# graphdeco-inria/reduced-3dgs

Measured on AMD Instinct MI355X. Metric: train iters/s (fwd+bwd) + Mpix/s render, 500k Gaussians @1600x1062, higher is better.
Workload: dtype f32

## Files before the change

reduced-3dgs_amd/csrc/binning.hip:

```cpp
#include <cstdlib>
#include <cstring>
#include <mutex>
#include <string>

#include <rocprim/rocprim.hpp>

#include "depth_sort.h"

namespace r3 {

struct GatherTiles {
    const uint32_t* tiles;
    __host__ __device__ uint32_t operator()(uint32_t id) const { return tiles[id]; }
};

size_t depth_sort_temp_bytes(size_t P)
{
    size_t a = 0, b = 0;
    uint32_t* n = nullptr;
    R3_HIP(rocprim::radix_sort_pairs(nullptr, a, n, n, rocprim::counting_iterator<uint32_t>(0), n, P, 0, 32));
    auto it = rocprim::make_transform_iterator(n, GatherTiles{n});
    R3_HIP(rocprim::inclusive_scan(nullptr, b, it, n, P, rocprim::plus<uint32_t>()));
    return (a > b ? a : b) + 256;
}

void run_generic_depth_sort(int P, GeomState& g, hipStream_t s)
{
    size_t bytes = g.temp_bytes;
    R3_HIP(rocprim::radix_sort_pairs(g.temp, bytes, g.depth_key, g.key_sorted, rocprim::counting_iterator<uint32_t>(0),
                                     g.order, (size_t)P, 0, 32, s));
    bytes = g.temp_bytes;
    auto it = rocprim::make_transform_iterator(g.order, GatherTiles{g.tiles});
    R3_HIP(rocprim::inclusive_scan(g.temp, bytes, it, g.offsets, (size_t)P, rocprim::plus<uint32_t>(), s));
}

__global__ __launch_bounds__(1024) void header_reduce_kernel(const HeaderArgs* __restrict__ ap)
{
    __shared__ uint32_t s_red[16][6];
    const HeaderArgs a = *ap;
    const PrePartial all = reduce_partials(a.parts, a.n_parts, s_red);
    if (threadIdx.x == 0) write_header(a, all);
}
// ... 124 lines not shown
    const uint32_t n = min(j_hi - j_lo + 1u, (uint32_t)kEmitSlice);
    const uint32_t start0 = s_start0;
    auto stage = [&](uint32_t r0, uint32_t nr) {
        for (uint32_t k = threadIdx.x; k < nr; k += 256) {
            const uint32_t g = j_lo + r0 + k, id = a.order[g];
            s_start[k] = r0 + k == 0 ? start0 : offsets[g - 1];
            s_id[k] = id;
            s_rect[k] = a.rect_sorted ? a.rect_sorted[g] : a.rect[id];
        }
    };
    const uint32_t nr0 = min(n, (uint32_t)kEmitStage);
    stage(0u, nr0);
    __syncthreads();
    for (uint32_t k = threadIdx.x; k < n; k += 256) {
        const uint32_t start = k < nr0 ? s_start[k] : offsets[j_lo + k - 1];
        a.rec[k < nr0 ? s_id[k] : a.order[j_lo + k]].pair_start = start;
        if (start >= pos0) s_owner[start - pos0] = (unsigned short)k;
    }
    __syncthreads();
    {
        constexpr int E = kEmitPerBlock / 256;
        const int lane = threadIdx.x & 63, w = threadIdx.x >> 6;
        uint32_t v[E];
#pragma unroll
        for (int i = 0; i < E; i++) v[i] = s_owner[threadIdx.x * E + i];
#pragma unroll
        for (int i = 1; i < E; i++) v[i] = max(v[i], v[i - 1]);
        uint32_t incl = v[E - 1];
        for (int off = 1; off < 64; off <<= 1) {
            const uint32_t up = (uint32_t)__shfl_up((int)incl, off);
            if (lane >= off) incl = max(incl, up);
// ... 354 lines not shown
```

reduced-3dgs_amd/csrc/blend.hip:

```cpp
#include <cstdlib>

#include "blend_math.h"
#include "common.h"

namespace r3 {

constexpr int kChunk = 64;

#if defined(R3_TIMELINE) || defined(R3_TIMELINE_FWD)
__device__ unsigned long long g_timeline[4 * 65536];
#define R3_TL_BEGIN_(id) const unsigned long long tl0_ = __builtin_amdgcn_s_memtime(); const uint32_t tlid_ = (id);
#define R3_TL_END_(extra)                                                                                                \
    if (threadIdx.x == 0 && tlid_ < 65536u) {                                                                            \
        g_timeline[4 * tlid_] = tl0_;                                                                                     \
        g_timeline[4 * tlid_ + 1] = __builtin_amdgcn_s_memtime();                                                         \
        g_timeline[4 * tlid_ + 2] = (unsigned long long)__builtin_amdgcn_s_getreg((4 << 0) | (0 << 6) | (31 << 11)) |     \
                                    ((unsigned long long)__builtin_amdgcn_s_getreg((20 << 0) | (0 << 6) | (31 << 11)) << 32); \
        g_timeline[4 * tlid_ + 3] = (unsigned long long)(extra);                                                          \
    }
#endif
#if defined(R3_TIMELINE)
#define R3_TL_BEGIN(id) R3_TL_BEGIN_(id)
#define R3_TL_END(extra) R3_TL_END_(extra)
#else
// ... 533 lines not shown
                {
                    typedef float v4f __attribute__((ext_vector_type(4)));
                    const volatile v4f __attribute__((address_space(3)))* zp =
                        (const volatile v4f __attribute__((address_space(3)))*)reinterpret_cast<float*>(s_zero);
                    const v4f z0 = zp[0], z1 = zp[1];
                    const float z2 = *(const volatile float __attribute__((address_space(3)))*)(zp + 2);
                    sg.sx = z0.x; sg.sy = z0.y; sg.sxx = z0.z; sg.sxy = z0.w;
                    sg.syy = z1.x; sg.sm = z1.y; sg.r = z1.z; sg.g = z1.w; sg.b = z2;
                }
#else
                sg.sx = sg.sy = sg.sxx = sg.sxy = sg.syy = sg.sm = sg.r = sg.g = sg.b = 0.f;
#endif
            }
        }
        __syncthreads();
        if (lane < n && ((contributed >> lane) & 1ull)) {
            const float4 c = s_rec[lane].c;
            const uint32_t rect_min = __float_as_uint(c.y), width = __float_as_uint(c.z) & 0xffffu;
            const uint32_t slot = __float_as_uint(c.w) + ((uint32_t)tile_y - (rect_min >> 16)) * width +
                                  ((uint32_t)tile_x - (rect_min & 0xffffu));
            float4* dst = reinterpret_cast<float4*>(a.pair_grad + (size_t)slot * kPairStride);
            const float* src = s_grad + lane * kGradStride;
            SplatSums u;
            u.sx = src[0];
            u.sy = src[1];
            u.sxx = src[2];
            u.sxy = src[3];
            u.syy = src[4];
            u.sm = src[5];
            u.r = src[6];
            u.g = src[7];
            u.b = src[8];
            const SplatGrad g = splat_grad_of(load_splat(s_rec[lane]), u);
            dst[0] = make_float4(g.mx * half_w, g.my * half_h, g.cA, g.cB);
            dst[1] = make_float4(g.cC, g.op, g.r, g.g);
            dst[2] = make_float4(g.b, 0.f, 0.f, 0.f);
            if (kPairStride >= 16) dst[3] = make_float4(0.f, 0.f, 0.f, 0.f);
            a.pair_flag[slot] = 1;
        }
    }
    R3_TL_END(hi - lo)
}

#if defined(R3_TIMELINE) || defined(R3_TIMELINE_FWD)
extern "C" int r3dgs_debug_timeline(unsigned long long* host, int n)
{
    return (int)hipMemcpyFromSymbol(host, HIP_SYMBOL(g_timeline), sizeof(unsigned long long) * 4 * (size_t)n);
}
#endif

constexpr int kOrderThreads = 1024, kOrderClasses = 1024;

__device__ __forceinline__ uint32_t unit_segments(uint32_t list_len, uint32_t deepest, uint32_t thr, uint32_t walk)
// ... 254 lines not shown
```

reduced-3dgs_amd/csrc/capi.hip:

```cpp
#include "../../include/r3dgs_rasterizer.h"
#include "../../include/r3dgs_quantised.h"

#include <time.h>

#include <atomic>
#include <random>
#include <chrono>
#include <cmath>
#include <cstddef>
#include <cstdlib>
#include <cstring>
#include <deque>
#include <map>
#include <mutex>
#include <unordered_map>
#include <vector>

#include "common.h"
#include "quant_math.h"

namespace r3 {
int env_int(const char* env, int dflt, int lo, int hi)
{
    const char* v = getenv(env);
// ... 397 lines not shown
    }
}

template <class Block>
void launch_write_args(Block* dst, const Block& v, hipStream_t s);

template <class Hooks>
void issue_backward(const BwdPlan& p, BwdPassArgs* d, const BwdPassArgs& args, hipStream_t s, Hooks& h)
{
    h.begin(kBlendBwd, s);
    if (p.has_pairs) {
        issue_unit_order(p, d, args, s);
        h.begin(kBlendBwdKernel, s);
        issue_blend_backward(p, d, args, s);
        h.end(kBlendBwdKernel, "blend backward kernel", s);
        issue_pair_reduce(p, &d->reduce, s);
    } else {
        launch_write_args(d, args, s);
    }
    h.end(kBlendBwd, "blend backward", s);
    h.begin(kPreBwd, s);
    issue_preprocess_backward(p, &d->pre, s);
    h.end(kPreBwd, "preprocess backward", s);
}

template <class Block>
void launch_write_args(Block* dst, const Block& v, hipStream_t s)
{
    hipLaunchKernelGGL(write_args_kernel<Block>, dim3(1), dim3(256), 0, s, dst, v);
}

// ... 193 lines not shown
    d.hist_rows = g.hist_rows;
    d.hist_base = g.hist_base;
    d.key_sorted = g.key_sorted;
    d.bucket_id = g.bucket_id;
    d.ovf_key = g.ovf_key;
    d.ovf_id = g.ovf_id;
    d.rect = g.rect;
    d.rec16 = g.rec16;
    d.rec16_b = g.rec16_b;
    d.rect_sorted = g.rect_sorted;
    d.order = g.order;
    d.offsets = g.offsets;
    uint32_t* const block_first = (b && fuse_header && !p.generic_depth_sort) ? b->block_first : nullptr;
    d.block_first = block_first;
    d.block_cap = p.reserve / (uint32_t)kRadixBlock + 2u;

    const PairLayout& l = p.layout;
    const size_t Tn = (size_t)p.gx * p.gy;
    if (b) {
        const uint32_t stride = radix_row_stride(p.reserve);
        EmitArgs& e = a.emit;
        e.P = c.P;
        e.gx = p.gx;
        e.hdr = g.header;
        e.order = g.order;
        e.offsets = g.offsets;
        e.block_first = block_first;
        e.rect = g.rect;
        e.rect_sorted = p.generic_depth_sort ? nullptr : g.rect_sorted;
        e.rec = g.rec;
// ... 539 lines not shown
        bb.W = width;
        bb.H = height;
        bb.gx = plan.gx;
        bb.nblocks = (uint32_t)(plan.gx * plan.gy * (4 / plan.bwd_ppl));
        bb.bg = background;
        bb.pair_grad = bin.pair_grad;
        bb.pair_flag = bin.pair_flag;
        bb.quad_masks = binning_buffer && keep_quad_masks() ? bin.quad_masks : nullptr;
        bb.tile_order = (heaviest_tiles_first() && plan.has_pairs && (size_t)plan.gx * plan.gy <= ((size_t)1 << kUnitTileBits))
                            ? bin.unit_order : nullptr;
        bb.units_cap = plan.units_cap;
        bb.quad_depth = img.quad_depth;
        bb.ckpt = plan.has_pairs ? bin.ckpt : nullptr;
        bb.hdr = geom.header;
        bb.segments = bwd_segments();
        PairReduceArgs& pr = a.reduce;
        pr.hdr = geom.header;
        pr.pair_grad = bin.pair_grad;
        pr.pair_flag = bin.pair_flag;
        pr.pair_rank = bin.pair_rank;
        pr.rank_mask = plan.layout.wide ? 0xFFFFFFFFu : (1u << plan.layout.rank_bits) - 1u;
        pr.order = nullptr;
        pr.rec = geom.rec;
        pr.tiles = geom.tiles;
        pr.acc = geom.acc;
        pr.wave_part = bin.wave_part;
        {
            static std::atomic<unsigned long long> stamp{[] {
                std::random_device rd;
                return ((unsigned long long)rd() << 32) ^ (unsigned long long)rd() ^ 0x9E3779B97F4A7C15ull;
            }()};
            const unsigned long long st = stamp.fetch_add(1);
            pr.stamp0 = (uint32_t)st;
            pr.stamp1 = (uint32_t)(st >> 32);
        }
        PreBwdArgs& pb = a.pre;
        FwdInputs& in = pb.in;
        in.P = P;
        in.M = M;
        in.degrees = D;
        in.means3D = means3D;
        in.scales = scales;
        in.rotations = rotations;
        in.opacities = nullptr;
        in.shs = colors_precomp ? nullptr : shs;
        in.cov3D_precomp = cov3D_precomp;
        in.colors_precomp = colors_precomp;
        ViewParams& view = pb.view;
        view.view = viewmatrix;
        view.proj = projmatrix;
        view.campos = campos;
        view.bg = background;
        view.tan_fovx = tan_fovx;
        view.tan_fovy = tan_fovy;
        view.W = width;
        view.H = height;
        view.scale_modifier = scale_modifier;
        pb.radii = radii;
        pb.rec = geom.rec;
        pb.tiles = geom.tiles;
        pb.acc = geom.acc;
        pb.wave_part = plan.has_pairs ? bin.wave_part : nullptr;
        pb.stamp0 = pr.stamp0;
        pb.stamp1 = pr.stamp1;
        pb.header = geom.header;
        pb.lambda_sh = lambda_sh_sparsity;
        pb.sh_ddir = (lambda_sh_sparsity == 0.f && sh_derivative_cache()) ? geom.sh_ddir : nullptr;
        pb.out.dL_dmean2D = dL_dmean2D;
        pb.out.dL_dopacity = dL_dopacity;
        pb.out.dL_dcolor = dL_dcolor;
        pb.out.dL_dmean3D = dL_dmean3D;
        pb.out.dL_dcov3D = dL_dcov3D;
        pb.out.dL_dsh = dL_dsh;
        pb.shs_rest = raw ? shs_rest : nullptr;
        pb.dL_dsh_rest = raw ? dL_dsh_rest : nullptr;
        pb.out.dL_dscale = dL_dscale;
        pb.out.dL_drot = dL_drot;
        pb.out.dL_dconic = dL_dconic;
        {
// ... 331 lines not shown
```

reduced-3dgs_amd/csrc/common.h:

```cpp
#pragma once
#include <hip/hip_runtime.h>
#include <stddef.h>
#include <stdint.h>

#include <functional>
#include <stdexcept>
#include <string>

#include "gauss_math.h"
#include "param_math.h"

namespace r3 {

constexpr size_t kAlign = 256;
constexpr int kPairGrad = 9;
constexpr int kPieceStride = 9;
constexpr int kAccStride = 12;
constexpr int kPairStride = 12;
static_assert(kAccStride >= 12 && kAccStride % 4 == 0 && kPairStride >= 12 && kPairStride % 4 == 0,
              "the kernels move three float4 per row");

constexpr int kPreBlockSize = 256;
struct PrePartial {
    uint32_t visible;
    uint32_t num_rendered;
    uint32_t depth_max;
    uint32_t depth_inv_min;
    uint32_t binned;
    uint32_t rendered_ref;
    uint32_t pad[2];
};
static_assert(sizeof(PrePartial) == 32, "two 16-byte loads per partial");
struct GeomHeader {
    uint32_t visible, num_rendered, depth_max, depth_inv_min;
    uint32_t num_pairs;
// ... 60 lines not shown
    {
        T* r = reinterpret_cast<T*>(p);
        size_t bytes = (count * sizeof(T) + kAlign - 1) & ~(kAlign - 1);
        p += bytes;
        return r;
    }
};

struct GeomState {
    GeomHeader* header;
    PrePartial* partials;
    DepthSortScratch* dsort;
    unsigned long long* hist_rows;
    uint32_t* hist_base;
    GRec* rec;
    float* acc;
    ushort4* rect;
    uint32_t* depth_key;
    uint32_t* tiles;
    uint32_t* key_sorted;
    uint32_t* bucket_id;
    uint4* rec16;
    ushort4* rect_sorted;
    uint4* rec16_b;
    uint32_t* order;
    uint32_t* offsets;
    int* radii_internal;
    float* sh_ddir;
    uint32_t* ovf_key;
    uint32_t* ovf_id;
    char* temp;
    size_t temp_bytes;
    static GeomState carve(char* base, size_t P, size_t temp_bytes)
    {
        Carver c(base);
        GeomState g;
        const size_t nb = (size_t)depth_bucket_count(P);
        g.header = c.take<GeomHeader>(1);
        g.partials = c.take<PrePartial>(pre_partials(P));
        g.dsort = c.take<DepthSortScratch>(1);
        g.hist_rows = c.take<unsigned long long>(depth_hist_rows(P) * (nb + 1));
        g.hist_base = c.take<uint32_t>(depth_hist_rows(P) * (nb + 1));
        g.rec = c.take<GRec>(P);
        g.acc = c.take<float>(P * kAccStride);
        g.rect = c.take<ushort4>(P);
        g.depth_key = c.take<uint32_t>(P);
        g.tiles = c.take<uint32_t>(P);
        g.key_sorted = c.take<uint32_t>(P);
        g.bucket_id = c.take<uint32_t>(P);
        g.order = c.take<uint32_t>(P);
        g.offsets = c.take<uint32_t>(P);
        g.radii_internal = c.take<int>(P);
        g.ovf_key = c.take<uint32_t>(P);
        g.ovf_id = c.take<uint32_t>(P);
        g.rec16 = c.take<uint4>(P);
        g.rect_sorted = c.take<ushort4>(P);
        g.rec16_b = c.take<uint4>(P);
        g.temp = c.take<char>(temp_bytes);
        g.temp_bytes = temp_bytes;
// ... 66 lines not shown
        return (uint32_t)(m < n() ? m : n());
    }
};
R3_HD uint32_t bwd_list_fit(uint32_t pairs, const TileGrid& g)
{
    const size_t extra = (size_t)pairs >> kBwdSegMinLog2, most = 8 * g.n();
    return g.list_tiles_max() + (uint32_t)((extra < most ? extra : most) / kOrderLists);
}
inline uint32_t bwd_units_cap(uint32_t reserve, const TileGrid& g) { return (bwd_list_fit(reserve, g) + 1u) * kOrderLists; }
int bwd_segment_log2();
int bwd_segment_factor_pct();

struct BinState {
    uint32_t* point_list;
    float* pair_grad;
    float* wave_part;
    unsigned char* pair_flag;
    uint32_t* pair_rank;
    char* words_a;
    char* words_b;
    char* words_c;
    uint32_t* radix_rows;
    uint32_t* radix_base;
    uint32_t* radix_total;
    uint32_t* block_first;
    unsigned long long* quad_masks;
    uint32_t* unit_order;
    float4* ckpt;
    char* end;
    static BinState carve(char* base, size_t R, int wide, const TileGrid& grid)
    {
        const size_t Tn = grid.n();
        Carver c(base);
        BinState b;
        b.point_list = c.take<uint32_t>(R);
        b.pair_grad = c.take<float>(R * kPairStride);
        b.wave_part = c.take<float>((R / 64 + 1) * 2 * kPieceStride);
        b.pair_flag = c.take<unsigned char>(R);
        if (wide == 1) {
            b.pair_rank = c.take<uint32_t>(R);
            b.words_a = reinterpret_cast<char*>(c.take<unsigned long long>(R));
            b.words_b = reinterpret_cast<char*>(c.take<unsigned long long>(R));
            b.words_c = nullptr;
        } else if (wide == 2) {
            b.words_a = reinterpret_cast<char*>(c.take<unsigned long long>(R));
            b.words_b = reinterpret_cast<char*>(c.take<unsigned long long>(R));
            b.words_c = nullptr;
            b.pair_rank = reinterpret_cast<uint32_t*>(b.words_a);
        } else {
            b.words_a = reinterpret_cast<char*>(c.take<uint32_t>(R));
            b.words_b = reinterpret_cast<char*>(c.take<uint32_t>(R));
            b.words_c = reinterpret_cast<char*>(c.take<uint32_t>(R));
// ... 193 lines not shown
    DepthSortScratch* ds;
    unsigned long long* hist_rows;
    uint32_t* hist_base;
    uint32_t* key_sorted;
    uint32_t* bucket_id;
    uint32_t* ovf_key;
    uint32_t* ovf_id;
    const ushort4* rect;
    uint4* rec16;
    uint4* rec16_b;
    ushort4* rect_sorted;
    uint32_t* order;
    uint32_t* offsets;
    uint32_t* block_first;
    uint32_t block_cap;
};
struct EmitArgs {
    int P, gx;
    const GeomHeader* hdr;
    const uint32_t* order;
    const uint32_t* offsets;
    const uint32_t* block_first;
    const ushort4* rect;
    const ushort4* rect_sorted;
    GRec* rec;
    int rank_bits, digit_bits;
    char* words_out;
    uint32_t cap;
    uint32_t* pair_rank;
    uint2* ranges;
// ... 49 lines not shown
    const uint32_t* n_contrib;
    const float* dL_dpix;
    int W, H, gx;
    uint32_t nblocks;
    const float* bg;
    float* pair_grad;
    unsigned char* pair_flag;
    const unsigned long long* quad_masks;
    uint32_t* tile_order;
    uint32_t units_cap;
    const uint32_t* quad_depth;
    const float4* ckpt;
    const GeomHeader* hdr;
    int segments;
};
struct PairReduceArgs {
    const GeomHeader* hdr;
    const float* pair_grad;
    unsigned char* pair_flag;
    const uint32_t* pair_rank;
    uint32_t rank_mask;
    const uint32_t* order;
    const GRec* rec;
    const uint32_t* tiles;
    float* acc;
    float* wave_part;
    uint32_t stamp0, stamp1;
};
struct PreBwdArgs {
    FwdInputs in;
    ViewParams view;
    const int* radii;
    const GRec* rec;
    const uint32_t* tiles;
    const float* acc;
    const float* wave_part;
    uint32_t stamp0, stamp1;
    const GeomHeader* header;
    float lambda_sh;
    const float* sh_ddir;
    int stagger;
    BwdOutputs out;
    const float* shs_rest;
    float* dL_dsh_rest;
};

struct FwdPassArgs {
    PreArgs pre;
    HeaderArgs header;
    DepthArgs depth;
    EmitArgs emit;
    RadixArgs radix[kMaxRadixPasses];
    RangesArgs ranges;
    BlendFwdArgs blend;
    const float* shs_rest;
    QuantInputs quant;
};
struct BwdPassArgs {
    BlendBwdArgs blend;
    PairReduceArgs reduce;
    PreBwdArgs pre;
};
static_assert(sizeof(FwdPassArgs) <= 3072 && sizeof(BwdPassArgs) <= 3072, "pass blocks travel as by-value kernel arguments");

struct FwdPlan {
    int P, M, W, H, gx, gy;
    uint32_t reserve;
    uint32_t grid_pairs;
    PairLayout layout;
    int nb;
    int ragged, counters;
    int color_grid;
    int color_split[3];
    int generic_depth_sort;
    int tight;
// ... 24 lines not shown
                             int* degrees, hipStream_t s);

void issue_header_reduce(const HeaderArgs* a, hipStream_t s);
void prepare_depth_bucket_sort(int nb);
void issue_depth_sort_and_color(const FwdPlan& p, const FwdPassArgs* a, hipStream_t s);
void run_generic_depth_sort(int P, GeomState& g, hipStream_t s);
void issue_tile_binning(const FwdPlan& p, const FwdPassArgs* a, hipStream_t s);
const char* sorted_words(const BinState& b, const PairLayout& l);
void launch_export_keys(int P, int R, int cap, size_t n_tiles, const BinState& b, const GeomState& g, uint64_t* keys_out,
                        hipStream_t s);
void launch_export_point_list(int count, const uint32_t* point_list, const GeomHeader* hdr, uint32_t* out, hipStream_t s);

void issue_blend_forward(const FwdPlan& p, const BlendFwdArgs* a, hipStream_t s);
void issue_unit_order(const BwdPlan& p, BwdPassArgs* dst, const BwdPassArgs& v, hipStream_t s);
void issue_blend_backward(const BwdPlan& p, BwdPassArgs* dst, const BwdPassArgs& v, hipStream_t s);
void issue_pair_reduce(const BwdPlan& p, const PairReduceArgs* a, hipStream_t s);
void issue_preprocess_backward(const BwdPlan& p, const PreBwdArgs* a, hipStream_t s);

void launch_colour_variance_accumulate(int P, const int* D, int M, int max_sh_deg, const float* means3D,
                                       const float* cam_pos, const float* shs, const int* radii, const int* touched,
                                       const float* transmittance, float* wSum, float* wSumSq, float* mean,
                                       float* variance, float* accum, hipStream_t s);

int env_int(const char* env, int dflt, int lo, int hi);

#if defined(__HIPCC__)
template <class Block>
__device__ __forceinline__ void install_block_from_kernarg(Block* dst, int tid, int nthreads)
{
    static_assert(alignof(Block) == 8 && sizeof(Block) % 4 == 0, "kernarg layout: [dst (8 B)][block]");
#if defined(__HIP_DEVICE_COMPILE__)
// ... 10 lines not shown
```

reduced-3dgs_amd/csrc/depth_sort.h:

```cpp
#pragma once
#include "common.h"

namespace r3 {

template <class T>
__device__ inline T block256_inclusive_scan(T v, T* s_w)
{
    const int lane = threadIdx.x & 63, w = threadIdx.x >> 6;
    for (int off = 1; off < 64; off <<= 1) {
        const T up = __shfl_up(v, off);
        if (lane >= off) v += up;
    }
    __syncthreads();
    if (lane == 63) s_w[w] = v;
    __syncthreads();
    T add = 0;
    for (int k = 0; k < w; k++) add += s_w[k];
    return v + add;
}

template <int BITS>
__device__ __forceinline__ unsigned long long match_digit(uint32_t d, bool valid)
{
    unsigned long long peers = __ballot(valid);
#pragma unroll
    for (int b = 0; b < BITS; b++) {
        const bool bit = (d >> b) & 1u;
        const unsigned long long bal = __ballot(bit);
        peers &= bit ? bal : ~bal;
    }
    return peers;
}

constexpr int kWaveSortMax = 512;
constexpr int kGlobalSplitMax = 64;
constexpr uint32_t kGlobalSplitCap = kGlobalSplitMax * 2048u;
constexpr int kBucketsPerGroup = 4;
constexpr int kHistPerThread = kHistBatch / 256;
constexpr int kCountBits = 24;
constexpr unsigned long long kCountMask = (1ull << kCountBits) - 1;

__device__ __forceinline__ void publish_offset(const DepthArgs& a, uint32_t slot, uint32_t end, uint32_t count)
{
    a.offsets[slot] = end;
    if (a.block_first && count) {
        const uint32_t first = end - count;
        for (uint32_t m = (first + (uint32_t)kRadixBlock - 1u) / (uint32_t)kRadixBlock;
// ... 203 lines not shown
    unsigned long long run = block256_inclusive_scan(sum, s_tmp) - sum;
    for (int k = 0; k < per; k++) {
        const int b = b0 + k;
        if (b <= nb + 1) {
            s_start[b] = (uint32_t)(run & kCountMask);
            if (publish) {
                ds->start[b] = (uint32_t)(run & kCountMask);
                ds->tile_base[b] = (uint32_t)(run >> kCountBits);
            }
            run += b <= nb ? ds->total[b] : 0ull;
        }
    }
    __syncthreads();
}

__device__ inline void depth_scatter_role(const DepthArgs& a, char* smem, int wg)
{
    const int P = a.P, nb = a.nb;
    unsigned long long* s_tmp = reinterpret_cast<unsigned long long*>(smem);
    uint32_t* slot0 = reinterpret_cast<uint32_t*>(smem + 256 * sizeof(unsigned long long));
    uint32_t* rank = slot0 + (nb + 2);
    scan_bucket_totals(a.ds, nb, slot0, s_tmp, wg == 0);
    if (wg == 0 && threadIdx.x == 0 && a.info) {
        volatile PassInfo* info = a.info;
        info->sort_overflow = a.hdr->sort_overflow;
        __threadfence_system();
        info->sort_seq = a.ticket;
    }
    const uint32_t R = a.hdr->num_rendered;
    const uint32_t* mybase = a.hist_base + (size_t)wg * (nb + 1);
    for (int b = threadIdx.x; b <= nb; b += 256) {
        slot0[b] += mybase[b];
        rank[b] = 0;
    }
    const DepthRange rng = make_depth_range(a.hdr->depth_max, a.hdr->depth_inv_min, nb);
    __syncthreads();
    const uint2* __restrict__ rects = reinterpret_cast<const uint2*>(a.rect);
    for (int base = wg * a.per_block; base < min(P, (wg + 1) * a.per_block); base += kHistBatch) {
        uint32_t kv[kHistPerThread];
        uint2 rv[kHistPerThread];
#pragma unroll
        for (int k = 0; k < kHistPerThread; k++) {
            const int i = base + k * 256 + threadIdx.x;
            kv[k] = i < P ? a.key[i] : 0xFFFFFFFFu;
            rv[k] = i < P ? rects[i] : make_uint2(0u, 0u);
        }
#pragma unroll
        for (int k = 0; k < kHistPerThread; k++) {
            const uint32_t id = (uint32_t)(base + k * 256 + threadIdx.x);
            if ((int)id < P) {
                const int b = depth_bucket(kv[k], rng);
                const uint32_t slot = slot0[b] + atomicAdd(&rank[b], 1u);
                if (b == nb) {
                    a.order[slot] = id;
                    a.offsets[slot] = R;
                } else {
                    a.rec16[slot] = make_uint4(kv[k], id, rv[k].x, rv[k].y);
                }
            }
        }
// ... 482 lines not shown
```

reduced-3dgs_amd/csrc/preprocess_bwd.hip:

```cpp
#include "common.h"

namespace r3 {

constexpr int kBwdBlock = 64;
constexpr int kBwdWaveShFloats = 64 * 48 + (64 * 48) / 32;

template <bool ROWS48>
__device__ __forceinline__ int bskew(int e)
{
    if (ROWS48) return e + (int)(((uint32_t)e * 43691u) >> 21);
    return e + (e >> 5);
}

template <bool ROWS48>
struct ShRowLdsRW {
    float* base;
    int roff;
    __device__ __forceinline__ float at(int e) const { return ROWS48 ? base[e] : base[bskew<false>(roff + e)]; }
    __device__ __forceinline__ void put(int e, float v) const
    {
        if (ROWS48)
            base[e] = v;
        else
            base[bskew<false>(roff + e)] = v;
// ... 55 lines not shown
            for (int e4 = lane; e4 < n4; e4 += 64) {
                const int f = e4 << 2;
                dst4[e4] = make_float4(lds[split_lds_index<ROWS48>(f, rl, k0, M)], lds[split_lds_index<ROWS48>(f + 1, rl, k0, M)],
                                       lds[split_lds_index<ROWS48>(f + 2, rl, k0, M)], lds[split_lds_index<ROWS48>(f + 3, rl, k0, M)]);
            }
        } else {
            for (int e4 = lane; e4 < n4; e4 += 64) dst4[e4] = make_float4(0.f, 0.f, 0.f, 0.f);
        }
    } else if (rows) {
        for (int f = lane; f < len; f += 64) dst[f] = lds[split_lds_index<ROWS48>(f, rl, k0, M)];
    } else {
        for (int f = lane; f < len; f += 64) dst[f] = 0.f;
    }
}

constexpr int kReduceGroups = 1;

__device__ __forceinline__ void pair_reduce_group(const PairReduceArgs& a, uint32_t e, int lane, bool valid, uint32_t key,
                                                  float (&v)[kPairGrad], uint32_t key_before, uint32_t key_after)
{
#define R3_SEG_STEP(CTRL, RMASK)                                                                                          \
    {                                                                                                                     \
        const uint32_t ku = (uint32_t)__builtin_amdgcn_update_dpp((int)~key, (int)key, CTRL, RMASK, 0xf, false);          \
        const bool take = ku == key;                                                                                      \
        _Pragma("unroll") for (int k = 0; k < kPairGrad; k++)                                                             \
        {                                                                                                                 \
            const float vu = __builtin_bit_cast(                                                                          \
                float, __builtin_amdgcn_update_dpp(0, __builtin_bit_cast(int, v[k]), CTRL, RMASK, 0xf, false));           \
            if (take) v[k] += vu;                                                                                         \
        }                                                                                                                 \
    }
    R3_SEG_STEP(0x111, 0xf)
    R3_SEG_STEP(0x112, 0xf)
    R3_SEG_STEP(0x114, 0xf)
    R3_SEG_STEP(0x118, 0xf)
    R3_SEG_STEP(0x142, 0xa)
    R3_SEG_STEP(0x143, 0xc)
#undef R3_SEG_STEP
    const uint32_t knext = (uint32_t)__shfl_down((int)key, 1);
    const uint32_t key0 = (uint32_t)__builtin_amdgcn_readfirstlane((int)key);
    if (valid && (lane == 63 || knext != key)) {
        const uint32_t gid = a.order ? global_ptr(a.order)[key] : key;
        const bool from_before = key == key0 && key_before == key;
        const bool into_next = lane == 63 && key_after == key;
        if (!from_before && !into_next) {
            auto* dst = reinterpret_cast<R3_GLOBAL float4*>(global_ptr(a.acc) + (size_t)gid * kAccStride);
            bool nz = false;
#pragma unroll
            for (int k = 0; k < kPairGrad; k++) nz |= v[k] != 0.f;
            if (nz) {
                dst[0] = make_float4(v[0], v[1], v[2], v[3]);
                dst[1] = make_float4(v[4], v[5], v[6], v[7]);
                dst[2] = make_float4(v[8], __uint_as_float(a.stamp0), __uint_as_float(a.stamp1), 0.f);
            }
        } else {
            R3_GLOBAL float* wp = global_ptr(a.wave_part) + (size_t)(e >> 6) * 2 * kPieceStride;
            if (from_before) {
#pragma unroll
                for (int k = 0; k < kPairGrad; k++) wp[k] = v[k];
            }
            if (into_next) {
#pragma unroll
                for (int k = 0; k < kPairGrad; k++) wp[kPieceStride + k] = v[k];
            }
        }
    }
}

__global__ __launch_bounds__(256) void pair_reduce_kernel(const PairReduceArgs* __restrict__ ap)
{
    const PairReduceArgs a = *ap;
    const uint32_t R = global_ptr(a.hdr)->num_pairs;
    constexpr uint32_t kPerBlock = 256u * kReduceGroups;
  for (uint32_t blk = blockIdx.x; blk * kPerBlock < R; blk += gridDim.x) {
    const R3_GLOBAL float* __restrict__ pair_grad = global_ptr(a.pair_grad);
    R3_GLOBAL unsigned char* __restrict__ pair_flag = global_ptr(a.pair_flag);
    const R3_GLOBAL uint32_t* __restrict__ pair_gid = global_ptr(a.pair_rank);
    const uint32_t rank_mask = a.rank_mask;
    const int lane = threadIdx.x & 63, wave = threadIdx.x >> 6;
    const uint32_t e0 = blk * kPerBlock + (uint32_t)wave * (64u * kReduceGroups) + (uint32_t)lane;
    float v[kReduceGroups][kPairGrad];
    uint32_t key[kReduceGroups], kb[kReduceGroups], ka[kReduceGroups];
    bool flag[kReduceGroups];
#pragma unroll
    for (int g = 0; g < kReduceGroups; g++) {
        const uint32_t e = e0 + 64u * g, gbase = e & ~63u;
        key[g] = e < R ? pair_gid[e] & rank_mask : 0xFFFFFFFFu;
        flag[g] = e < R && pair_flag[e] != 0;
        kb[g] = gbase > 0u && gbase < R ? pair_gid[gbase - 1u] & rank_mask : 0xFFFFFFFFu;
        ka[g] = gbase + 64u < R ? pair_gid[gbase + 64u] & rank_mask : 0xFFFFFFFFu;
    }
#pragma unroll
    for (int g = 0; g < kReduceGroups; g++) {
        const uint32_t e = e0 + 64u * g;
#pragma unroll
        for (int k = 0; k < kPairGrad; k++) v[g][k] = 0.f;
        if (flag[g]) {
            pair_flag[e] = 0;
            const auto* src = reinterpret_cast<const R3_GLOBAL float4*>(pair_grad + (size_t)e * kPairStride);
            const float4 r0 = src[0], r1 = src[1];
            v[g][0] = r0.x; v[g][1] = r0.y; v[g][2] = r0.z; v[g][3] = r0.w;
            v[g][4] = r1.x; v[g][5] = r1.y; v[g][6] = r1.z; v[g][7] = r1.w;
            v[g][8] = src[2].x;
        }
    }
#pragma unroll
    for (int g = 0; g < kReduceGroups; g++) {
        const uint32_t e = e0 + 64u * g;
        pair_reduce_group(a, e, lane, e < R, key[g], v[g], kb[g], ka[g]);
    }
  }
}

void issue_pair_reduce(const BwdPlan& p, const PairReduceArgs* a, hipStream_t s)
{
    if (!p.has_pairs) return;
    constexpr uint32_t per = 256u * kReduceGroups;
    hipLaunchKernelGGL(pair_reduce_kernel, dim3((p.grid_pairs + per - 1u) / per), dim3(256), 0, s, a);
}

template <bool ROWS48, bool F64, bool RAW = false>
__global__ __launch_bounds__(kBwdBlock) void preprocess_bwd_kernel(const PreBwdArgs* __restrict__ ap)
{
    __shared__ float s_sh[kBwdBlock / 64][kBwdWaveShFloats];
    const PreBwdArgs a = *ap;
    const int tid = threadIdx.x, lane = tid & 63, wave = tid >> 6;
    const int P = a.in.P, M = a.in.M;
    const int i = blockIdx.x * kBwdBlock + tid;
    const bool valid = i < P;
    const int wave_first = blockIdx.x * kBwdBlock + wave * 64;
    const Camera cam = load_camera_from(global_ptr(a.view.view), global_ptr(a.view.proj), global_ptr(a.view.campos), a.view);
    const bool has_sh = a.in.shs != nullptr;
    const auto* hdr = global_ptr(a.header);
    const uint32_t num_pairs = hdr->num_pairs, n_visible = hdr->visible, hdr_sh_cache = hdr->sh_cache;
    const bool cached = has_sh && a.sh_ddir != nullptr && hdr_sh_cache != 0u;

    int radius = 0, deg = 0;
    uint32_t ntile = 0u;
    GRec r;
    float4 a0, a1, a2;
    float m3[3], sc[3], q[4], c6[6], d9in[9];
    const auto load_lane = [&]() {
        r = global_ptr(a.rec)[i];
        ntile = global_ptr(a.tiles)[i];
        const auto* arow = reinterpret_cast<const R3_GLOBAL float4*>(global_ptr(a.acc) + (size_t)i * kAccStride);
        a0 = arow[0];
        a1 = arow[1];
        a2 = arow[2];
        for (int k = 0; k < 3; k++) m3[k] = global_ptr(a.in.means3D)[3 * i + k];
        if (!a.in.cov3D_precomp) {
            for (int k = 0; k < 3; k++) sc[k] = global_ptr(a.in.scales)[3 * i + k];
            for (int k = 0; k < 4; k++) q[k] = global_ptr(a.in.rotations)[4 * i + k];
        }
        if (has_sh) deg = global_ptr(a.in.degrees)[i];
        if (cached) {
#pragma unroll
            for (int k = 0; k < 9; k++) d9in[k] = global_ptr(a.sh_ddir)[9 * (size_t)i + k];
        }
        if (a.in.cov3D_precomp) {
            for (int k = 0; k < 6; k++) c6[k] = global_ptr(a.in.cov3D_precomp)[6 * i + k];
            sc[0] = sc[1] = sc[2] = 0.f;
            q[0] = 1.f;
            q[1] = q[2] = q[3] = 0.f;
        }
    };
    if (valid) radius = global_ptr(a.radii)[i];
    const bool vis = valid && radius > 0;
    if (vis) load_lane();

    const int nrows = max(0, min(64, P - wave_first));
    const int span_len = has_sh ? nrows * 3 * M : 0;
    const long span_first = 3L * M * wave_first;
    float* lds = s_sh[wave];
    const bool wave_vis = __ballot(vis) != 0ull;
    if (!cached && a.stagger > 0 && blockIdx.x < 768u * (256 / kBwdBlock)) {
        const int steps = (int)(blockIdx.x / (256u * (256 / kBwdBlock))) * a.stagger;
        for (int k = 0; k < steps; k += 127) __builtin_amdgcn_s_sleep(127);
    }
    if (RAW) {
        if (wave_vis && !cached) {
            const int rl = 3 * (M - 1);
            const auto* dc = global_ptr(a.in.shs) + 3L * wave_first;
            const auto* rest = global_ptr(a.shs_rest) + (long)rl * wave_first;
// ... 40 lines not shown
                }
            }
        } else {
            for (int e = lane; e < span_len; e += 64) lds[bskew<ROWS48>(e)] = src[e];
        }
    }
    __syncthreads();

    float dmean[3] = {0.f, 0.f, 0.f}, dcov6[6] = {0.f, 0.f, 0.f, 0.f, 0.f, 0.f};
    float dscale[3] = {0.f, 0.f, 0.f}, dq[4] = {0.f, 0.f, 0.f, 0.f};
    float g2x = 0.f, g2y = 0.f, dop = 0.f, dcol[3] = {0.f, 0.f, 0.f}, gcon[3] = {0.f, 0.f, 0.f};
    int K = 0;
    const ShRowLdsRW<ROWS48> row{ROWS48 ? lds + 49 * lane : lds, ROWS48 ? 0 : lane * 3 * M};
    if (vis) {
        const float mx = m3[0], my = m3[1], mz = m3[2];
        const uint32_t start = r.pair_start;
        if (a.wave_part && start != 0xFFFFFFFFu && start + ntile <= num_pairs) {
            float acc9[kPairGrad];
            const uint32_t last = start + ntile - 1u;
            const uint32_t w0 = start >> 6, w1 = last >> 6;
            if (w0 == w1) {
                if (__float_as_uint(a2.y) != a.stamp0 || __float_as_uint(a2.z) != a.stamp1)
                    a0 = a1 = a2 = make_float4(0.f, 0.f, 0.f, 0.f);
                acc9[0] = a0.x; acc9[1] = a0.y; acc9[2] = a0.z; acc9[3] = a0.w;
                acc9[4] = a1.x; acc9[5] = a1.y; acc9[6] = a1.z; acc9[7] = a1.w;
                acc9[8] = a2.x;
            } else {
                const R3_GLOBAL float* wave_part = global_ptr(a.wave_part);
                const R3_GLOBAL float* wp = wave_part + (size_t)w0 * 2 * kPieceStride + kPieceStride;
#pragma unroll
                for (int k = 0; k < kPairGrad; k++) acc9[k] = wp[k];
                for (uint32_t w = w0 + 1; w <= w1; w++) {
                    wp = wave_part + (size_t)w * 2 * kPieceStride;
#pragma unroll
                    for (int k = 0; k < kPairGrad; k++) acc9[k] += wp[k];
                }
            }
            g2x = acc9[0];
            g2y = acc9[1];
            gcon[0] = acc9[2];
            gcon[1] = acc9[3];
            gcon[2] = acc9[4];
            dop = acc9[5];
            dcol[0] = acc9[6];
            dcol[1] = acc9[7];
            dcol[2] = acc9[8];
        }
        float qn = 1.f;
        if (!a.in.cov3D_precomp) {
            if (RAW) {
                const float rq[4] = {q[0], q[1], q[2], q[3]};
                for (int k = 0; k < 3; k++) sc[k] = scale_act(sc[k]);
                qn = quat_act(rq, q);
            }
            cov3d_from_scale_rot(sc, cam.scale_modifier, q, c6);
        }
        double dcov6d[6];
        if (F64) {
            cov2d_backward_f64(cam, mx, my, mz, c6, gcon[0], gcon[1], gcon[2], dcov6d, dmean);
#pragma unroll
            for (int k = 0; k < 6; k++) dcov6[k] = (float)dcov6d[k];
        } else {
// ... 141 lines not shown
```

Baseline: 1588.

## Fold per-pair gradient reduction into preprocess backward via slab-ordered pair layout

Removes the separate pair_reduce kernel and its per-Gaussian acc buffer, wave_part spill and stamp scheme. Pair slots are now assigned in Gaussian-index order: a prefix scan over tile counts runs inside the depth scatter, or in two extra kernels on the generic sort path. Each preprocess-backward wave then reads its contiguous slab of pair gradients directly and reduces them with segmented shuffles. This removes a kernel launch and a global round trip, but adds scan work to binning and reduction work inside the backward preprocess. Reading pair gradients in Gaussian order may also change the access locality of the blend writes.

After: 1577. About the same (-0.7%).

```diff
diff --git a/reduced-3dgs_amd/csrc/binning.hip b/reduced-3dgs_amd/csrc/binning.hip
--- a/reduced-3dgs_amd/csrc/binning.hip
+++ b/reduced-3dgs_amd/csrc/binning.hip
@@ -24,8 +24,49 @@
     return (a > b ? a : b) + 256;
 }
 
+__global__ __launch_bounds__(1024) void slab_part_scan_kernel(const PrePartial* __restrict__ parts, int n, uint32_t* __restrict__ out)
+{
+    __shared__ uint32_t s_w[16];
+    const int lane = threadIdx.x & 63, w = threadIdx.x >> 6;
+    uint32_t run = 0u;
+    for (int base = 0; base < n; base += 1024) {
+        const int j = base + (int)threadIdx.x;
+        const uint32_t v = j < n ? parts[j].num_rendered : 0u;
+        const uint32_t incl = wave_inclusive_scan(v, lane);
+        __syncthreads();
+        if (lane == 63) s_w[w] = incl;
+        __syncthreads();
+        uint32_t add = run, total = 0u;
+        for (int k = 0; k < 16; k++) {
+            if (k < w) add += s_w[k];
+            total += s_w[k];
+        }
+        if (j < n) out[j] = add + incl - v;
+        run += total;
+    }
+}
+__global__ __launch_bounds__(kPreBlockSize) void slab_start_kernel(int P, const uint32_t* __restrict__ part_start,
+                                                                   const uint32_t* __restrict__ tiles,
+                                                                   const uint32_t* __restrict__ key, GRec* __restrict__ rec,
+                                                                   uint32_t* __restrict__ slab_wave)
+{
+    __shared__ uint32_t s_w[4];
+    const int i = (int)blockIdx.x * kPreBlockSize + (int)threadIdx.x, lane = threadIdx.x & 63;
+    const uint32_t t = i < P ? tiles[i] : 0u;
+    const uint32_t incl = block256_inclusive_scan(t, s_w);
+    if (i < P) {
+        const uint32_t start = part_start[blockIdx.x] + incl - t;
+        if (key[i] != 0xFFFFFFFFu) rec[i].pair_start = start;
+        if (lane == 0) slab_wave[i >> 6] = start;
+    }
+}
+
 void run_generic_depth_sort(int P, GeomState& g, hipStream_t s)
 {
+    const int n_parts = (int)pre_partials((size_t)P);
+    hipLaunchKernelGGL(slab_part_scan_kernel, dim3(1), dim3(1024), 0, s, g.partials, n_parts, g.slab_part);
+    hipLaunchKernelGGL(slab_start_kernel, dim3(n_parts), dim3(kPreBlockSize), 0, s, P, g.slab_part, g.tiles, g.depth_key, g.rec,
+                       g.slab_wave);
     size_t bytes = g.temp_bytes;
     R3_HIP(rocprim::radix_sort_pairs(g.temp, bytes, g.depth_key, g.key_sorted, rocprim::counting_iterator<uint32_t>(0),
                                      g.order, (size_t)P, 0, 32, s));
@@ -180,7 +221,6 @@
     __syncthreads();
     for (uint32_t k = threadIdx.x; k < n; k += 256) {
         const uint32_t start = k < nr0 ? s_start[k] : offsets[j_lo + k - 1];
-        a.rec[k < nr0 ? s_id[k] : a.order[j_lo + k]].pair_start = start;
         if (start >= pos0) s_owner[start - pos0] = (unsigned short)k;
     }
     __syncthreads();
diff --git a/reduced-3dgs_amd/csrc/blend.hip b/reduced-3dgs_amd/csrc/blend.hip
--- a/reduced-3dgs_amd/csrc/blend.hip
+++ b/reduced-3dgs_amd/csrc/blend.hip
@@ -571,6 +571,7 @@
             }
         }
         __syncthreads();
+        const uint32_t slab_end = contributed ? a.hdr->num_pairs : 0u;
         if (lane < n && ((contributed >> lane) & 1ull)) {
             const float4 c = s_rec[lane].c;
             const uint32_t rect_min = __float_as_uint(c.y), width = __float_as_uint(c.z) & 0xffffu;
@@ -589,11 +590,13 @@
             u.g = src[7];
             u.b = src[8];
             const SplatGrad g = splat_grad_of(load_splat(s_rec[lane]), u);
-            dst[0] = make_float4(g.mx * half_w, g.my * half_h, g.cA, g.cB);
-            dst[1] = make_float4(g.cC, g.op, g.r, g.g);
-            dst[2] = make_float4(g.b, 0.f, 0.f, 0.f);
-            if (kPairStride >= 16) dst[3] = make_float4(0.f, 0.f, 0.f, 0.f);
-            a.pair_flag[slot] = 1;
+            if (slot < slab_end) {
+                dst[0] = make_float4(g.mx * half_w, g.my * half_h, g.cA, g.cB);
+                dst[1] = make_float4(g.cC, g.op, g.r, g.g);
+                dst[2] = make_float4(g.b, 0.f, 0.f, 0.f);
+                if (kPairStride >= 16) dst[3] = make_float4(0.f, 0.f, 0.f, 0.f);
+                a.pair_flag[slot] = 1;
+            }
         }
     }
     R3_TL_END(hi - lo)
diff --git a/reduced-3dgs_amd/csrc/capi.hip b/reduced-3dgs_amd/csrc/capi.hip
--- a/reduced-3dgs_amd/csrc/capi.hip
+++ b/reduced-3dgs_amd/csrc/capi.hip
@@ -4,7 +4,6 @@
 #include <time.h>
 
 #include <atomic>
-#include <random>
 #include <chrono>
 #include <cmath>
 #include <cstddef>
@@ -435,7 +434,6 @@
         h.begin(kBlendBwdKernel, s);
         issue_blend_backward(p, d, args, s);
         h.end(kBlendBwdKernel, "blend backward kernel", s);
-        issue_pair_reduce(p, &d->reduce, s);
     } else {
         launch_write_args(d, args, s);
     }
@@ -659,6 +657,9 @@
     uint32_t* const block_first = (b && fuse_header && !p.generic_depth_sort) ? b->block_first : nullptr;
     d.block_first = block_first;
     d.block_cap = p.reserve / (uint32_t)kRadixBlock + 2u;
+    d.parts = g.partials;
+    d.rec = g.rec;
+    d.slab_wave = g.slab_wave;
 
     const PairLayout& l = p.layout;
     const size_t Tn = (size_t)p.gx * p.gy;
@@ -1228,26 +1229,6 @@
         bb.ckpt = plan.has_pairs ? bin.ckpt : nullptr;
         bb.hdr = geom.header;
         bb.segments = bwd_segments();
-        PairReduceArgs& pr = a.reduce;
-        pr.hdr = geom.header;
-        pr.pair_grad = bin.pair_grad;
-        pr.pair_flag = bin.pair_flag;
-        pr.pair_rank = bin.pair_rank;
-        pr.rank_mask = plan.layout.wide ? 0xFFFFFFFFu : (1u << plan.layout.rank_bits) - 1u;
-        pr.order = nullptr;
-        pr.rec = geom.rec;
-        pr.tiles = geom.tiles;
-        pr.acc = geom.acc;
-        pr.wave_part = bin.wave_part;
-        {
-            static std::atomic<unsigned long long> stamp{[] {
-                std::random_device rd;
-                return ((unsigned long long)rd() << 32) ^ (unsigned long long)rd() ^ 0x9E3779B97F4A7C15ull;
-            }()};
-            const unsigned long long st = stamp.fetch_add(1);
-            pr.stamp0 = (uint32_t)st;
-            pr.stamp1 = (uint32_t)(st >> 32);
-        }
         PreBwdArgs& pb = a.pre;
         FwdInputs& in = pb.in;
         in.P = P;
@@ -1273,10 +1254,9 @@
         pb.radii = radii;
         pb.rec = geom.rec;
         pb.tiles = geom.tiles;
-        pb.acc = geom.acc;
-        pb.wave_part = plan.has_pairs ? bin.wave_part : nullptr;
-        pb.stamp0 = pr.stamp0;
-        pb.stamp1 = pr.stamp1;
+        pb.pair_grad = plan.has_pairs ? bin.pair_grad : nullptr;
+        pb.pair_flag = plan.has_pairs ? bin.pair_flag : nullptr;
+        pb.slab_wave = geom.slab_wave;
         pb.header = geom.header;
         pb.lambda_sh = lambda_sh_sparsity;
         pb.sh_ddir = (lambda_sh_sparsity == 0.f && sh_derivative_cache()) ? geom.sh_ddir : nullptr;
diff --git a/reduced-3dgs_amd/csrc/common.h b/reduced-3dgs_amd/csrc/common.h
--- a/reduced-3dgs_amd/csrc/common.h
+++ b/reduced-3dgs_amd/csrc/common.h
@@ -14,11 +14,8 @@
 
 constexpr size_t kAlign = 256;
 constexpr int kPairGrad = 9;
-constexpr int kPieceStride = 9;
-constexpr int kAccStride = 12;
 constexpr int kPairStride = 12;
-static_assert(kAccStride >= 12 && kAccStride % 4 == 0 && kPairStride >= 12 && kPairStride % 4 == 0,
-              "the kernels move three float4 per row");
+static_assert(kPairStride >= 12 && kPairStride % 4 == 0, "the kernels move three float4 per row");
 
 constexpr int kPreBlockSize = 256;
 struct PrePartial {
@@ -109,7 +106,8 @@
     unsigned long long* hist_rows;
     uint32_t* hist_base;
     GRec* rec;
-    float* acc;
+    uint32_t* slab_wave;
+    uint32_t* slab_part;
     ushort4* rect;
     uint32_t* depth_key;
     uint32_t* tiles;
@@ -137,7 +135,8 @@
         g.hist_rows = c.take<unsigned long long>(depth_hist_rows(P) * (nb + 1));
         g.hist_base = c.take<uint32_t>(depth_hist_rows(P) * (nb + 1));
         g.rec = c.take<GRec>(P);
-        g.acc = c.take<float>(P * kAccStride);
+        g.slab_wave = c.take<uint32_t>((P + 63) / 64);
+        g.slab_part = c.take<uint32_t>(pre_partials(P));
         g.rect = c.take<ushort4>(P);
         g.depth_key = c.take<uint32_t>(P);
         g.tiles = c.take<uint32_t>(P);
@@ -234,7 +233,6 @@
 struct BinState {
     uint32_t* point_list;
     float* pair_grad;
-    float* wave_part;
     unsigned char* pair_flag;
     uint32_t* pair_rank;
     char* words_a;
@@ -255,7 +253,6 @@
         BinState b;
         b.point_list = c.take<uint32_t>(R);
         b.pair_grad = c.take<float>(R * kPairStride);
-        b.wave_part = c.take<float>((R / 64 + 1) * 2 * kPieceStride);
         b.pair_flag = c.take<unsigned char>(R);
         if (wide == 1) {
             b.pair_rank = c.take<uint32_t>(R);
@@ -479,6 +476,9 @@
     uint32_t* offsets;
     uint32_t* block_first;
     uint32_t block_cap;
+    const PrePartial* parts;
+    GRec* rec;
+    uint32_t* slab_wave;
 };
 struct EmitArgs {
     int P, gx;
@@ -558,28 +558,15 @@
     const GeomHeader* hdr;
     int segments;
 };
-struct PairReduceArgs {
-    const GeomHeader* hdr;
-    const float* pair_grad;
-    unsigned char* pair_flag;
-    const uint32_t* pair_rank;
-    uint32_t rank_mask;
-    const uint32_t* order;
-    const GRec* rec;
-    const uint32_t* tiles;
-    float* acc;
-    float* wave_part;
-    uint32_t stamp0, stamp1;
-};
 struct PreBwdArgs {
     FwdInputs in;
     ViewParams view;
     const int* radii;
     const GRec* rec;
     const uint32_t* tiles;
-    const float* acc;
-    const float* wave_part;
-    uint32_t stamp0, stamp1;
+    const float* pair_grad;
+    unsigned char* pair_flag;
+    const uint32_t* slab_wave;
     const GeomHeader* header;
     float lambda_sh;
     const float* sh_ddir;
@@ -602,7 +589,6 @@
 };
 struct BwdPassArgs {
     BlendBwdArgs blend;
-    PairReduceArgs reduce;
     PreBwdArgs pre;
 };
 static_assert(sizeof(FwdPassArgs) <= 3072 && sizeof(BwdPassArgs) <= 3072, "pass blocks travel as by-value kernel arguments");
@@ -657,7 +643,6 @@
 void issue_blend_forward(const FwdPlan& p, const BlendFwdArgs* a, hipStream_t s);
 void issue_unit_order(const BwdPlan& p, BwdPassArgs* dst, const BwdPassArgs& v, hipStream_t s);
 void issue_blend_backward(const BwdPlan& p, BwdPassArgs* dst, const BwdPassArgs& v, hipStream_t s);
-void issue_pair_reduce(const BwdPlan& p, const PairReduceArgs* a, hipStream_t s);
 void issue_preprocess_backward(const BwdPlan& p, const PreBwdArgs* a, hipStream_t s);
 
 void launch_colour_variance_accumulate(int P, const int* D, int M, int max_sh_deg, const float* means3D,
diff --git a/reduced-3dgs_amd/csrc/depth_sort.h b/reduced-3dgs_amd/csrc/depth_sort.h
--- a/reduced-3dgs_amd/csrc/depth_sort.h
+++ b/reduced-3dgs_amd/csrc/depth_sort.h
@@ -31,6 +31,8 @@
     }
     return peers;
 }
+
+__device__ __forceinline__ uint32_t wave_inclusive_scan(uint32_t v, int lane);
 
 constexpr int kWaveSortMax = 512;
 constexpr int kGlobalSplitMax = 64;
@@ -264,9 +266,23 @@
     __syncthreads();
 }
 
+static_assert(kHistBatch % kPreBlockSize == 0, "a scatter batch starts at a preprocess workgroup's first Gaussian");
+static_assert(kHistBatch / 256 * 4 == 64, "one wave scans the batch's (round, wave) totals");
 __device__ inline void depth_scatter_role(const DepthArgs& a, char* smem, int wg)
 {
+    __shared__ uint32_t s_slab[kHistPerThread * 4 + 1];
     const int P = a.P, nb = a.nb;
+    const int lane = threadIdx.x & 63, wv = threadIdx.x >> 6;
+    uint32_t slab_run = 0u;
+    {
+        const int first = (int)(((long long)wg * a.per_block) / kPreBlockSize);
+        for (int j = threadIdx.x; j < first; j += 256) slab_run += a.parts[j].num_rendered;
+        for (int off = 32; off > 0; off >>= 1) slab_run += (uint32_t)__shfl_xor((int)slab_run, off);
+        if (lane == 0) s_slab[wv] = slab_run;
+        __syncthreads();
+        slab_run = s_slab[0] + s_slab[1] + s_slab[2] + s_slab[3];
+        __syncthreads();
+    }
     unsigned long long* s_tmp = reinterpret_cast<unsigned long long*>(smem);
     uint32_t* slot0 = reinterpret_cast<uint32_t*>(smem + 256 * sizeof(unsigned long long));
     uint32_t* rank = slot0 + (nb + 2);
@@ -289,11 +305,39 @@
     for (int base = wg * a.per_block; base < min(P, (wg + 1) * a.per_block); base += kHistBatch) {
         uint32_t kv[kHistPerThread];
         uint2 rv[kHistPerThread];
+        uint32_t tv[kHistPerThread];
 #pragma unroll
         for (int k = 0; k < kHistPerThread; k++) {
             const int i = base + k * 256 + threadIdx.x;
             kv[k] = i < P ? a.key[i] : 0xFFFFFFFFu;
             rv[k] = i < P ? rects[i] : make_uint2(0u, 0u);
+            tv[k] = i < P ? a.tiles[i] : 0u;
+        }
+        {
+#pragma unroll
+            for (int k = 0; k < kHistPerThread; k++) {
+                const uint32_t incl = wave_inclusive_scan(tv[k], lane);
+                if (lane == 63) s_slab[k * 4 + wv] = incl;
+                tv[k] = incl - tv[k];
+            }
+            __syncthreads();
+            if (wv == 0) {
+                const uint32_t v = s_slab[lane], incl = wave_inclusive_scan(v, lane);
+                s_slab[lane] = incl - v;
+                if (lane == 63) s_slab[kHistPerThread * 4] = incl;
+            }
+            __syncthreads();
+#pragma unroll
+            for (int k = 0; k < kHistPerThread; k++) {
+                const int i = base + k * 256 + (int)threadIdx.x;
+                if (i < P) {
+                    const uint32_t start = slab_run + s_slab[k * 4 + wv] + tv[k];
+                    if (kv[k] != 0xFFFFFFFFu) a.rec[i].pair_start = start;
+                    if (lane == 0) a.slab_wave[i >> 6] = start;
+                }
+            }
+            slab_run += s_slab[kHistPerThread * 4];
+            __syncthreads();
         }
 #pragma unroll
         for (int k = 0; k < kHistPerThread; k++) {
diff --git a/reduced-3dgs_amd/csrc/preprocess_bwd.hip b/reduced-3dgs_amd/csrc/preprocess_bwd.hip
--- a/reduced-3dgs_amd/csrc/preprocess_bwd.hip
+++ b/reduced-3dgs_amd/csrc/preprocess_bwd.hip
@@ -93,10 +93,18 @@
     }
 }
 
-constexpr int kReduceGroups = 1;
-
-__device__ __forceinline__ void pair_reduce_group(const PairReduceArgs& a, uint32_t e, int lane, bool valid, uint32_t key,
-                                                  float (&v)[kPairGrad], uint32_t key_before, uint32_t key_after)
+constexpr int kSlabGroups = 4;
+
+__device__ __forceinline__ uint32_t wave_inclusive_sum(uint32_t v, int lane)
+{
+    for (int off = 1; off < 64; off <<= 1) {
+        const uint32_t up = (uint32_t)__shfl_up((int)v, off);
+        if (lane >= off) v += up;
+    }
+    return v;
+}
+
+__device__ __forceinline__ void pair_reduce_group(uint32_t key, float (&v)[kPairGrad])
 {
 #define R3_SEG_STEP(CTRL, RMASK)                                                                                          \
     {                                                                                                                     \
@@ -116,86 +124,78 @@
     R3_SEG_STEP(0x142, 0xa)
     R3_SEG_STEP(0x143, 0xc)
 #undef R3_SEG_STEP
-    const uint32_t knext = (uint32_t)__shfl_down((int)key, 1);
-    const uint32_t key0 = (uint32_t)__builtin_amdgcn_readfirstlane((int)key);
-    if (valid && (lane == 63 || knext != key)) {
-        const uint32_t gid = a.order ? global_ptr(a.order)[key] : key;
-        const bool from_before = key == key0 && key_before == key;
-        const bool into_next = lane == 63 && key_after == key;
-        if (!from_before && !into_next) {
-            auto* dst = reinterpret_cast<R3_GLOBAL float4*>(global_ptr(a.acc) + (size_t)gid * kAccStride);
-            bool nz = false;
-#pragma unroll
-            for (int k = 0; k < kPairGrad; k++) nz |= v[k] != 0.f;
-            if (nz) {
-                dst[0] = make_float4(v[0], v[1], v[2], v[3]);
-                dst[1] = make_float4(v[4], v[5], v[6], v[7]);
-                dst[2] = make_float4(v[8], __uint_as_float(a.stamp0), __uint_as_float(a.stamp1), 0.f);
-            }
-        } else {
-            R3_GLOBAL float* wp = global_ptr(a.wave_part) + (size_t)(e >> 6) * 2 * kPieceStride;
-            if (from_before) {
-#pragma unroll
-                for (int k = 0; k < kPairGrad; k++) wp[k] = v[k];
-            }
-            if (into_next) {
-#pragma unroll
-                for (int k = 0; k < kPairGrad; k++) wp[kPieceStride + k] = v[k];
-            }
-        }
-    }
-}
-
-__global__ __launch_bounds__(256) void pair_reduce_kernel(const PairReduceArgs* __restrict__ ap)
-{
-    const PairReduceArgs a = *ap;
-    const uint32_t R = global_ptr(a.hdr)->num_pairs;
-    constexpr uint32_t kPerBlock = 256u * kReduceGroups;
-  for (uint32_t blk = blockIdx.x; blk * kPerBlock < R; blk += gridDim.x) {
-    const R3_GLOBAL float* __restrict__ pair_grad = global_ptr(a.pair_grad);
-    R3_GLOBAL unsigned char* __restrict__ pair_flag = global_ptr(a.pair_flag);
-    const R3_GLOBAL uint32_t* __restrict__ pair_gid = global_ptr(a.pair_rank);
-    const uint32_t rank_mask = a.rank_mask;
-    const int lane = threadIdx.x & 63, wave = threadIdx.x >> 6;
-    const uint32_t e0 = blk * kPerBlock + (uint32_t)wave * (64u * kReduceGroups) + (uint32_t)lane;
-    float v[kReduceGroups][kPairGrad];
-    uint32_t key[kReduceGroups], kb[kReduceGroups], ka[kReduceGroups];
-    bool flag[kReduceGroups];
-#pragma unroll
-    for (int g = 0; g < kReduceGroups; g++) {
-        const uint32_t e = e0 + 64u * g, gbase = e & ~63u;
-        key[g] = e < R ? pair_gid[e] & rank_mask : 0xFFFFFFFFu;
-        flag[g] = e < R && pair_flag[e] != 0;
-        kb[g] = gbase > 0u && gbase < R ? pair_gid[gbase - 1u] & rank_mask : 0xFFFFFFFFu;
-        ka[g] = gbase + 64u < R ? pair_gid[gbase + 64u] & rank_mask : 0xFFFFFFFFu;
-    }
-#pragma unroll
-    for (int g = 0; g < kReduceGroups; g++) {
-        const uint32_t e = e0 + 64u * g;
-#pragma unroll
-        for (int k = 0; k < kPairGrad; k++) v[g][k] = 0.f;
-        if (flag[g]) {
-            pair_flag[e] = 0;
-            const auto* src = reinterpret_cast<const R3_GLOBAL float4*>(pair_grad + (size_t)e * kPairStride);
-            const float4 r0 = src[0], r1 = src[1];
-            v[g][0] = r0.x; v[g][1] = r0.y; v[g][2] = r0.z; v[g][3] = r0.w;
-            v[g][4] = r1.x; v[g][5] = r1.y; v[g][6] = r1.z; v[g][7] = r1.w;
-            v[g][8] = src[2].x;
-        }
-    }
-#pragma unroll
-    for (int g = 0; g < kReduceGroups; g++) {
-        const uint32_t e = e0 + 64u * g;
-        pair_reduce_group(a, e, lane, e < R, key[g], v[g], kb[g], ka[g]);
-    }
-  }
-}
-
-void issue_pair_reduce(const BwdPlan& p, const PairReduceArgs* a, hipStream_t s)
-{
-    if (!p.has_pairs) return;
-    constexpr uint32_t per = 256u * kReduceGroups;
-    hipLaunchKernelGGL(pair_reduce_kernel, dim3((p.grid_pairs + per - 1u) / per), dim3(256), 0, s, a);
+}
+
+__device__ __forceinline__ uint32_t slab_owner_lane(uint32_t end, uint32_t s)
+{
+    uint32_t cnt = 0u;
+#pragma unroll
+    for (uint32_t step = 32u; step > 0u; step >>= 1) {
+        const uint32_t e = (uint32_t)__shfl((int)end, (int)(cnt + step - 1u));
+        if (e <= s) cnt += step;
+    }
+    return cnt;
+}
+
+__device__ __forceinline__ void slab_reduce_wave(const R3_GLOBAL float* __restrict__ pair_grad,
+                                                 R3_GLOBAL unsigned char* __restrict__ pair_flag, uint32_t slab0,
+                                                 uint32_t num_pairs, uint32_t ntile, int lane, float (&sum)[kPairGrad])
+{
+    const uint32_t end = slab0 + wave_inclusive_sum(ntile, lane), start = end - ntile;
+    const uint32_t wave_end = (uint32_t)__builtin_amdgcn_readlane((int)end, 63);
+    const uint32_t read_end = min(wave_end, num_pairs);
+    uint32_t flag[kSlabGroups];
+#pragma unroll
+    for (int g = 0; g < kSlabGroups; g++) {
+        const uint32_t s = slab0 + 64u * g + (uint32_t)lane;
+        flag[g] = s < read_end ? (uint32_t)pair_flag[s] : 0u;
+    }
+    for (uint32_t b0 = slab0; b0 < read_end; b0 += 64u * kSlabGroups) {
+        float v[kSlabGroups][kPairGrad];
+        uint32_t next[kSlabGroups];
+#pragma unroll
+        for (int g = 0; g < kSlabGroups; g++) {
+            const uint32_t s = b0 + 64u * g + (uint32_t)lane;
+#pragma unroll
+            for (int k = 0; k < kPairGrad; k++) v[g][k] = 0.f;
+            if (flag[g]) {
+                const auto* src = reinterpret_cast<const R3_GLOBAL float4*>(pair_grad + (size_t)s * kPairStride);
+                const float4 r0 = src[0], r1 = src[1];
+                v[g][0] = r0.x; v[g][1] = r0.y; v[g][2] = r0.z; v[g][3] = r0.w;
+                v[g][4] = r1.x; v[g][5] = r1.y; v[g][6] = r1.z; v[g][7] = r1.w;
+                v[g][8] = src[2].x;
+                pair_flag[s] = 0;
+            }
+        }
+#pragma unroll
+        for (int g = 0; g < kSlabGroups; g++) {
+            const uint32_t s = b0 + 64u * (kSlabGroups + g) + (uint32_t)lane;
+            next[g] = s < read_end ? (uint32_t)pair_flag[s] : 0u;
+        }
+#pragma unroll
+        for (int g = 0; g < kSlabGroups; g++) {
+            const uint32_t g0 = b0 + 64u * g;
+            if (g0 < read_end) {
+                const uint32_t s = g0 + (uint32_t)lane;
+                const uint32_t owner = slab_owner_lane(end, s);
+                const uint32_t key = s < read_end ? owner : 0xFFFFFFFFu;
+                pair_reduce_group(key, v[g]);
+                const uint32_t lo = max(start, g0), hi = min(end, min(g0 + 64u, read_end));
+                const bool mine = lo < hi;
+                const int src_lane = (int)((hi - 1u - g0) & 63u);
+#pragma unroll
+                for (int k = 0; k < kPairGrad; k++) {
+                    const float part = __shfl(v[g][k], src_lane);
+                    if (mine) sum[k] += part;
+                }
+            }
+            flag[g] = next[g];
+        }
+    }
+    if (end > num_pairs) {
+#pragma unroll
+        for (int k = 0; k < kPairGrad; k++) sum[k] = 0.f;
+    }
 }
 
 template <bool ROWS48, bool F64, bool RAW = false>
@@ -217,15 +217,9 @@
     int radius = 0, deg = 0;
     uint32_t ntile = 0u;
     GRec r;
-    float4 a0, a1, a2;
     float m3[3], sc[3], q[4], c6[6], d9in[9];
     const auto load_lane = [&]() {
         r = global_ptr(a.rec)[i];
-        ntile = global_ptr(a.tiles)[i];
-        const auto* arow = reinterpret_cast<const R3_GLOBAL float4*>(global_ptr(a.acc) + (size_t)i * kAccStride);
-        a0 = arow[0];
-        a1 = arow[1];
-        a2 = arow[2];
         for (int k = 0; k < 3; k++) m3[k] = global_ptr(a.in.means3D)[3 * i + k];
         if (!a.in.cov3D_precomp) {
             for (int k = 0; k < 3; k++) sc[k] = global_ptr(a.in.scales)[3 * i + k];
@@ -243,9 +237,20 @@
             q[1] = q[2] = q[3] = 0.f;
         }
     };
-    if (valid) radius = global_ptr(a.radii)[i];
+    if (valid) {
+        radius = global_ptr(a.radii)[i];
+        ntile = global_ptr(a.tiles)[i];
+    }
     const bool vis = valid && radius > 0;
     if (vis) load_lane();
+
+    float acc9[kPairGrad];
+#pragma unroll
+    for (int k = 0; k < kPairGrad; k++) acc9[k] = 0.f;
+    if (a.pair_grad) {
+        const uint32_t slab0 = global_ptr(a.slab_wave)[blockIdx.x * (kBwdBlock / 64) + wave];
+        slab_reduce_wave(global_ptr(a.pair_grad), global_ptr(a.pair_flag), slab0, num_pairs, ntile, lane, acc9);
+    }
 
     const int nrows = max(0, min(64, P - wave_first));
     const int span_len = has_sh ? nrows * 3 * M : 0;
@@ -316,38 +321,15 @@
     const ShRowLdsRW<ROWS48> row{ROWS48 ? lds + 49 * lane : lds, ROWS48 ? 0 : lane * 3 * M};
     if (vis) {
         const float mx = m3[0], my = m3[1], mz = m3[2];
-        const uint32_t start = r.pair_start;
-        if (a.wave_part && start != 0xFFFFFFFFu && start + ntile <= num_pairs) {
-            float acc9[kPairGrad];
-            const uint32_t last = start + ntile - 1u;
-            const uint32_t w0 = start >> 6, w1 = last >> 6;
-            if (w0 == w1) {
-                if (__float_as_uint(a2.y) != a.stamp0 || __float_as_uint(a2.z) != a.stamp1)
-                    a0 = a1 = a2 = make_float4(0.f, 0.f, 0.f, 0.f);
-                acc9[0] = a0.x; acc9[1] = a0.y; acc9[2] = a0.z; acc9[3] = a0.w;
-                acc9[4] = a1.x; acc9[5] = a1.y; acc9[6] = a1.z; acc9[7] = a1.w;
-                acc9[8] = a2.x;
-            } else {
-                const R3_GLOBAL float* wave_part = global_ptr(a.wave_part);
-                const R3_GLOBAL float* wp = wave_part + (size_t)w0 * 2 * kPieceStride + kPieceStride;
-#pragma unroll
-                for (int k = 0; k < kPairGrad; k++) acc9[k] = wp[k];
-                for (uint32_t w = w0 + 1; w <= w1; w++) {
-                    wp = wave_part + (size_t)w * 2 * kPieceStride;
-#pragma unroll
-                    for (int k = 0; k < kPairGrad; k++) acc9[k] += wp[k];
-                }
-            }
-            g2x = acc9[0];
-            g2y = acc9[1];
-            gcon[0] = acc9[2];
-            gcon[1] = acc9[3];
-            gcon[2] = acc9[4];
-            dop = acc9[5];
-            dcol[0] = acc9[6];
-            dcol[1] = acc9[7];
-            dcol[2] = acc9[8];
-        }
+        g2x = acc9[0];
+        g2y = acc9[1];
+        gcon[0] = acc9[2];
+        gcon[1] = acc9[3];
+        gcon[2] = acc9[4];
+        dop = acc9[5];
+        dcol[0] = acc9[6];
+        dcol[1] = acc9[7];
+        dcol[2] = acc9[8];
         float qn = 1.f;
         if (!a.in.cov3D_precomp) {
             if (RAW) {
```
